# AnnaLew/pangenomix

Hardware: AMD Instinct MI355X
Metric: proteins/sec clustered at 0.8 identity + pan/core iters/sec, 400-genome set (higher is better)
Workload: dtype i32

## Files before the change

pangenomix_amd/csrc/cluster.hip:

```cpp
#include <algorithm>
#include <chrono>
#include <cstdlib>
#include <cmath>
#include <type_traits>
#include <functional>
#include <condition_variable>
#include <mutex>
#include <thread>
#include <vector>

#include "cluster_layout.h"
#include "cluster_resolve.h"
#include "cluster_tables.h"
#include "pgx_internal.h"

namespace {

using namespace pgxc;

constexpr uint32_t kWindowMax = 65536;
constexpr int kDiscoveryRounds = 2;
constexpr uint32_t kBlockCap = 4096;
constexpr uint32_t kBlockCapMin = 64;

constexpr uint32_t kMaxLen = 1u << 22;
constexpr uint32_t kPackedLenAa = 32767, kPackedLenNt = 16383;
constexpr uint32_t kSentinel = 0xFFFFFFFFu;
constexpr uint32_t kDiagLdsCap = 2048;
constexpr uint32_t kDiagLdsSmall = 512;
constexpr int kMaxBand = 64;

__constant__ int8_t kBlosum62_dev[kNAA1 * kNAA1] = PGXC_BLOSUM62_FLAT;

enum : uint32_t { E_TOUCHED = 1,
                  E_POOL = 2,
                  E_TABLE = 4,
                  E_BAND = 8,
                  E_PAIRS = 16,
                  E_WORDMULT = 32 };

struct PairSel {
    const uint32_t *d_begin, *d_end;
    uint32_t cap;
    const uint32_t *list;
    uint32_t n_list;
    const uint8_t *only_a, *only_not_b;
    uint8_t *accepted_out;
    uint32_t b0;
    uint32_t skip_evaluated;
    uint32_t all_if_le;
};
__device__ __forceinline__ uint32_t sel_count(const PairSel &s) {
    if (s.list) return s.n_list;
    uint32_t e = *s.d_end;
    if (e > s.cap) e = s.cap;
    const uint32_t b = s.d_begin ? *s.d_begin : 0u;
    return e > b ? e - b : 0u;
}
__device__ __forceinline__ uint32_t sel_pair(const PairSel &s, uint32_t w) {
    return s.list ? s.list[w] : (s.d_begin ? *s.d_begin : 0u) + w;
}

struct DevSeqs {
    const uint8_t *res;
    const uint64_t *off;
    const uint32_t *len;
    const uint32_t *wcode;
    const uint16_t *wmult;
    const uint32_t *wcnt;
    const uint32_t *pk;
    const uint32_t *pk_off;
    uint32_t n_fwd;
    int32_t base;
    int32_t kd;
    int32_t nt;
    uint32_t mshift;
};
__device__ __forceinline__ uint32_t entry_rmask(const DevSeqs &S) { return (1u << S.mshift) - 1u; }
__device__ __forceinline__ uint32_t entry_fmax(const DevSeqs &S) { return 0xFFFFFFFFu >> S.mshift; }
__device__ __forceinline__ uint32_t real_of(const DevSeqs &S, uint32_t k) { return k >= S.n_fwd ? k - S.n_fwd : k; }

__constant__ int8_t kAa2Idx_dev[26] = {0, 2, 4, 3, 6, 13, 7, 8, 9, 20, 11, 10, 12,
                                       2, 20, 14, 5, 1, 15, 16, 20, 19, 17, 20, 18, 6};

__device__ __forceinline__ bool is_letter(uint8_t ch) {
    ch &= 0xDF;
    return ch >= 'A' && ch <= 'Z';
}

__global__ __launch_bounds__(256) void seq_len_kernel(const uint8_t *__restrict__ res,
                                                     const uint64_t *__restrict__ off, uint32_t n, uint64_t total,
                                                     uint32_t *__restrict__ len) {
    const uint32_t lane = threadIdx.x & 63u;
    const uint32_t i = blockIdx.x * 4u + (threadIdx.x >> 6);
    if (i >= n) return;
    const uint64_t b = off[i], e = off[i + 1];
    uint32_t c = 0;
    const uint64_t a0 = b & ~3ull;
    for (uint64_t a = a0 + 4ull * lane; a < e; a += 256) {
        uint32_t word = 0;
        if (a + 4 <= total) word = *reinterpret_cast<const uint32_t *>(res + a);
        else for (uint64_t p = a; p < total; ++p) word |= (uint32_t)res[p] << (8 * (p - a));
#pragma unroll
        for (int t = 0; t < 4; ++t) {
            const uint64_t p = a + t;
            c += (p >= b && p < e) && is_letter((uint8_t)(word >> (8 * t)));
        }
    }
    for (int d = 32; d > 0; d >>= 1) c += __shfl_xor(c, d);
    if (lane == 0) len[i] = c;
}

__global__ __launch_bounds__(256) void encode_gather_kernel(const uint8_t *__restrict__ in,
                                                           const uint64_t *__restrict__ in_off,
                                                           const uint32_t *__restrict__ order,
                                                           const uint64_t *__restrict__ out_off,
                                                           uint8_t *__restrict__ out, uint32_t n, int nt) {
    const uint32_t lane = threadIdx.x & 63u;
    const uint32_t k = blockIdx.x * 4u + (threadIdx.x >> 6);
    if (k >= n) return;
    const uint32_t src = order[k];
    const uint64_t b = in_off[src], e = in_off[src + 1];
    uint64_t w = out_off[k];
    for (uint64_t q0 = b; q0 < e; q0 += 256) {
        uint8_t chs[4];
#pragma unroll
        for (int j = 0; j < 4; ++j) { const uint64_t p = q0 + 64u * j + lane; chs[j] = p < e ? in[p] : (uint8_t)0; }
#pragma unroll
        for (int j = 0; j < 4; ++j) {
            const uint8_t ch = chs[j];
            const bool ok = is_letter(ch);
            const unsigned long long m = __ballot(ok);
            if (ok) {
                const uint8_t up = ch & 0xDF;
                const uint8_t idx = nt ? (uint8_t)(up == 'A' ? 0 : up == 'C' ? 1 : up == 'G' ? 2 : (up == 'T' || up == 'U') ? 3 : 4)
                                       : (uint8_t)kAa2Idx_dev[up - 'A'];
                out[w + __popcll(m & ((1ull << lane) - 1ull))] = idx;
            }
            w += __popcll(m);
        }
    }
}

__global__ __launch_bounds__(256) void revcomp_kernel(uint8_t *__restrict__ res, const uint64_t *__restrict__ off,
                                                     const uint32_t *__restrict__ len, uint32_t n) {
    const uint32_t lane = threadIdx.x & 63u;
    const uint32_t k = blockIdx.x * 4u + (threadIdx.x >> 6);
    if (k >= n) return;
    const uint64_t src = off[k], dst = off[n + k];
    const uint32_t L = len[k];
    for (uint32_t i = lane; i < L; i += 64) {
        const uint8_t b = res[src + L - 1 - i];
        res[dst + i] = b < 4 ? (uint8_t)(3 - b) : b;
    }
}

__global__ __launch_bounds__(256) void pack5_kernel(const uint8_t *__restrict__ res, const uint64_t *__restrict__ off,
                                                   const uint32_t *__restrict__ len,
                                                   const uint32_t *__restrict__ pk_off, uint32_t n,
                                                   uint32_t *__restrict__ pk) {
    const uint32_t lane = threadIdx.x & 63u;
    const uint32_t k = blockIdx.x * 4u + (threadIdx.x >> 6);
    if (k >= n) return;
    const uint8_t *s = res + off[k];
    const uint32_t L = len[k], nw = (L + 5u) / 6u;
    uint32_t *dst = pk + pk_off[k];
    for (uint32_t w = lane; w < nw; w += 64) {
// ... 1070 lines not shown
    __shared__ uint32_t s_cnt[4][kMaxChunks];
    const uint32_t lane = threadIdx.x & 63u, n = *n_open;
    uint32_t *cnt = s_cnt[threadIdx.x >> 6];
    for (uint32_t w = blockIdx.x * 4 + (threadIdx.x >> 6); w < n; w += gridDim.x * 4) {
        const uint32_t k = ulist[w], ql = k - b0;
        if (decided[ql]) continue;
        const uint32_t c = chunk_of(C, ql);
        const int32_t t0 = req_aan[k];
        bool cand = false;
        for (uint32_t strand = 0; strand < (both ? 2u : 1u) && !cand; ++strand) {
            const uint32_t ks = strand ? S.n_fwd + k : k;
            const uint64_t o = S.off[ks];
            const uint32_t nw = S.wcnt[ks];
            if (lane < kMaxChunks) cnt[lane] = 0u;
            __builtin_amdgcn_fence(__ATOMIC_RELEASE, "workgroup");
            __builtin_amdgcn_wave_barrier();
            uint32_t sum = 0;
            for (uint32_t i = lane; i < nw; i += 64) {
                const uint32_t m = S.wmult[o + i];
                const uint32_t *rec = first + (size_t)S.wcode[o + i] * stride;
                for (uint32_t t4 = 0; t4 <= c; t4 += 4) {
                    uint32_t v[4];
                    if (stride >= 4) { const uint4 x = *reinterpret_cast<const uint4 *>(rec + t4); v[0] = x.x; v[1] = x.y; v[2] = x.z; v[3] = x.w; }
                    else { v[0] = rec[0]; v[1] = stride > 1 ? rec[1] : 0u; v[2] = 0u; v[3] = 0u; }
#pragma unroll
                    for (uint32_t j = 0; j < 4; ++j) {
                        const uint32_t t = t4 + j;
                        if (t > c || (v[j] >> 16) != epoch) continue;
                        if (t < c) atomicAdd(&cnt[t], m);
                        else if (65535u - (v[j] & 65535u) < ql) sum += m;
                    }
                }
            }
            for (int d = 32; d > 0; d >>= 1) sum += __shfl_xor(sum, d);
            __builtin_amdgcn_fence(__ATOMIC_RELEASE, "workgroup");
            __builtin_amdgcn_wave_barrier();
            __builtin_amdgcn_fence(__ATOMIC_ACQUIRE, "workgroup");
            uint32_t mx = lane < c ? cnt[lane] : 0u;
            mx = mx > sum ? mx : sum;
            for (int d = 32; d > 0; d >>= 1) { const uint32_t v = __shfl_xor(mx, d); mx = v > mx ? v : mx; }
            cand = mx != 0u && (int32_t)mx >= t0;
            __builtin_amdgcn_wave_barrier();
        }
        if (!cand && lane == 0) {
            done[ql] = 1;
            list[atomicAdd(n_list, 1u)] = k;
        }
    }
}

__global__ __launch_bounds__(256) void thresholds_kernel(const uint32_t *__restrict__ len, uint32_t n,
                                                        const int32_t *__restrict__ tab, uint32_t n_len,
                                                        int32_t *__restrict__ aa1, int32_t *__restrict__ aas,
                                                        int32_t *__restrict__ aan) {
    const uint32_t k = blockIdx.x * blockDim.x + threadIdx.x;
    if (k >= n) return;
    const uint32_t L = len[k];
    aa1[k] = tab[L]; aas[k] = tab[n_len + L]; aan[k] = tab[2 * n_len + L];
}


__global__ void retire_block_kernel(uint8_t *__restrict__ done, uint8_t *__restrict__ inblk, uint32_t nb, uint32_t final_,
                                    uint32_t *__restrict__ begin) {
    const uint32_t q = blockIdx.x * blockDim.x + threadIdx.x;
    if (q == 0 && begin) { begin[C_TOUCH] = 0u; begin[C_NK] = 0u; begin[C_EVAL0] = begin[C_NW]; }
    if (q < nb && inblk[q]) { done[q] = (uint8_t)final_; inblk[q] = 0; }
}
__global__ __launch_bounds__(256) void window_init_kernel(uint32_t *__restrict__ counters,
                                                         unsigned long long *__restrict__ best,
                                                         unsigned long long *__restrict__ rc_visits,
                                                         uint8_t *__restrict__ flags, uint32_t window_cap) {
    const uint32_t q = blockIdx.x * blockDim.x + threadIdx.x;
    if (q < C_COUNT && q != C_ERR) counters[q] = 0u;
    if (q >= window_cap) return;
    best[q] = kNoBest;
    if (rc_visits) rc_visits[q] = 0ull;
    if (q < 4 * window_cap / 8) reinterpret_cast<unsigned long long *>(flags)[q] = 0ull;
}

__global__ __launch_bounds__(256) void mark_absent_kernel(const uint8_t *__restrict__ taken, uint32_t nb,
                                                         uint8_t *__restrict__ done,
                                                         unsigned long long *__restrict__ best) {
    const uint32_t q = blockIdx.x * blockDim.x + threadIdx.x;
    if (q < nb && taken[q]) { done[q] = 2; best[q] = 0ull; }
}

__global__ __launch_bounds__(256) void min_rows_kernel(const unsigned long long *__restrict__ rows, uint32_t n_rows,
                                                      uint32_t row_stride, uint32_t n,
                                                      unsigned long long *__restrict__ out, uint32_t *__restrict__ err) {
    const uint32_t i = blockIdx.x * blockDim.x + threadIdx.x;
    if (i == 0) {
        uint32_t e = 0;
        for (uint32_t r = 0; r < n_rows; ++r) e |= (uint32_t)rows[(size_t)r * row_stride + PGX_EXCHANGE_KEYS];
        if (e) atomicOr(err, e);
    }
    if (i >= n) return;
    unsigned long long m = rows[i];
    for (uint32_t r = 1; r < n_rows; ++r) { const unsigned long long v = rows[(size_t)r * row_stride + i]; m = v < m ? v : m; }
    out[i] = m;
}

__global__ void exchange_prepare_kernel(const uint32_t *__restrict__ counters, uint32_t pair_cap,
                                        unsigned long long *__restrict__ send, uint32_t inject) {
    send[PGX_EXCHANGE_KEYS] = counters[C_ERR] | (counters[C_NW] > pair_cap ? (uint32_t)E_PAIRS : 0u) | inject;
}

constexpr uint32_t kPairWords = sizeof(Pair) / 4;
static_assert(sizeof(Pair) % 4 == 0, "pair records are published as dwords");
struct PubSeg { const uint32_t *src; uint32_t *dst; const uint32_t *count; uint32_t fixed, words, cap; };
constexpr int kPubSegs = 8;
struct PubArgs { PubSeg seg[kPubSegs]; int n; };
__global__ __launch_bounds__(256) void publish_kernel(PubArgs a) {
    for (int s = 0; s < a.n; ++s) {
        const PubSeg g = a.seg[s];
        uint32_t c = g.count ? *g.count : g.fixed;
        if (c > g.cap) c = g.cap;
        const uint32_t total = c * g.words;
        for (uint32_t i = blockIdx.x * blockDim.x + threadIdx.x; i < total; i += gridDim.x * blockDim.x) g.dst[i] = g.src[i];
    }
}

__global__ __launch_bounds__(256) void gather_pairs_kernel(const Pair *__restrict__ pairs,
                                                          const uint32_t *__restrict__ list, uint32_t n,
                                                          Pair *__restrict__ out) {
    const uint32_t i = blockIdx.x * blockDim.x + threadIdx.x;
    if (i < n) out[i] = pairs[list[i]];
}


__device__ __forceinline__ uint32_t wave_excl_scan(uint32_t v, uint32_t lane, uint32_t *total) {
    uint32_t x = v;
    for (int d = 1; d < 64; d <<= 1) {
        const uint32_t y = __shfl_up(x, d);
        if ((int)lane >= d) x += y;
    }
    *total = __shfl(x, 63);
    return x - v;
}

template <typename DiagPtr>
__device__ void band_from_histogram(DiagPtr d, int len1, int len2, int band_width, int required_aa1,
                                    double cluster_thd, int *best_sum, int *bl, int *bc, int *br) {
    const int lane = threadIdx.x & 63;
    const int nall = len1 + len2 - 1;
    const int band_b = required_aa1 - 1 >= 0 ? required_aa1 - 1 : 0;
    const int band_e = nall - band_b;
    const int band_m = band_b + band_width - 1 < band_e ? band_b + band_width - 1 : band_e;
    const int w = band_m - band_b + 1;
    const int T = band_e - band_m - 1 > 0 && w > 0 ? band_e - band_m - 1 : 0;
    using Cell = std::remove_cv_t<std::remove_reference_t<decltype(d[0])>>;
    constexpr int kHalf = (int)sizeof(Cell) * 4;
    auto hits = [&](int i) { return (int)(d[i] & ((Cell(1) << kHalf) - 1)); };
    auto weighted = [&](int i) { return (int)(d[i] >> kHalf); };
    auto wave_max = [&](int v) { for (int o = 32; o > 0; o >>= 1) v = max(v, __shfl_xor(v, o)); return v; };
    auto wave_min = [&](int v) { for (int o = 32; o > 0; o >>= 1) v = min(v, __shfl_xor(v, o)); return v; };
    auto wave_sum = [&](int v) { for (int o = 32; o > 0; o >>= 1) v += __shfl_xor(v, o); return v; };
    const int x0 = lane < w ? weighted(band_b + lane) : 0;
    const int score2_first = wave_sum(x0);
    int max_diag2 = wave_max(x0);
    int imax = max_diag2 > 0 ? wave_min(x0 == max_diag2 && lane < w ? band_b + lane : INT32_MAX) : 0;
    const int per = (T + 63) / 64;
    const int t_lo = 1 + lane * per, t_hi = min(T + 1, t_lo + per);
    auto window_at = [&](int t) {
        int sum = 0;
        for (int i = 0; i < w; ++i) sum += weighted(band_b + t + i);
        return sum;
    };
    int first = 0, local_max = INT32_MIN;
    if (t_lo < t_hi) {
        first = window_at(t_lo);
        int sc = first;
        local_max = sc;
        for (int t = t_lo + 1; t < t_hi; ++t) {
            sc += weighted(band_m + t) - weighted(band_b + t - 1);
            local_max = max(local_max, sc);
        }
    }
    int before = local_max;
    for (int o = 1; o < 64; o <<= 1) {
        const int up = __shfl_up(before, o);
        if (lane >= o) before = max(before, up);
    }
    before = __shfl_up(before, 1);
    before = max(lane == 0 ? INT32_MIN : before, score2_first);
    int last_t = 0, cand_val = 0, cand_t = INT32_MAX;
    if (t_lo < t_hi) {
        int sc = first, run = before;
        for (int t = t_lo; t < t_hi; ++t) {
            if (t > t_lo) sc += weighted(band_m + t) - weighted(band_b + t - 1);
            if (sc > run) {
                run = sc; last_t = t;
                const int v = weighted(band_m + t);
                if (v > cand_val) { cand_val = v; cand_t = t; }
            }
        }
    }
    const int best_t = wave_max(last_t);
    const int cand_best = wave_max(cand_val);
    if (cand_best > max_diag2) {
        max_diag2 = cand_best;
        imax = band_m + wave_min(cand_val == cand_best ? cand_t : INT32_MAX);
    }
    int from = band_b + best_t, end = band_m + best_t;
    int best_score = wave_sum(lane < w ? hits(from + lane) : 0);
    int mlen = imax;
    if (imax > len1) mlen = nall - imax;
    const int emax = (int)((1.0 - cluster_thd) * mlen) + 1;
    for (int j = from; j < imax; ++j) {
        const int s1 = hits(j);
        if ((imax - j) > emax || s1 < 1) { best_score -= s1; from++; } else break;
    }
    for (int j = end; j > imax; --j) {
        const int s1 = j >= band_b ? hits(j) : 0;
        if ((j - imax) > emax || s1 < 1) { best_score -= s1; end--; } else break;
    }
    *bl = from - len1 + 1; *br = end - len1 + 1; *bc = imax - len1 + 1; *best_sum = best_score;
}

__device__ __forceinline__ int kd_code(const DevSeqs &S, const uint8_t *__restrict__ s, int j, int *cpx) {
    int code = 0, c = 1;
    bool bad = false;
    for (int t = 0; t < S.kd; ++t) {
        const int r = s[j + t];
        bad |= r >= S.base;
        code = code * S.base + r;
        if (t) c += r != s[j + t - 1];
    }
    *cpx = c;
    return (S.nt && bad) ? -1 : code;
}

template <uint32_t CAP, typename Cell>
__global__ __launch_bounds__(64) void diag_kernel(DevSeqs S, const uint32_t *__restrict__ rep_seq,
                                                 Pair *__restrict__ pairs, PairSel sel,
                                                 const int32_t *__restrict__ req_aa1,
                                                 const int32_t *__restrict__ req_aas, int band_width,
                                                 double cluster_thd, uint32_t *__restrict__ gscratch,
                                                 uint32_t gscratch_stride, uint32_t gscratch_cells,
                                                 uint32_t *__restrict__ n_wide, uint32_t *__restrict__ err) {
    if (blockIdx.x == 0 && threadIdx.x == 0) *n_wide = 0u;
    constexpr bool kWideCell = sizeof(Cell) == 8;
    constexpr int kHalf = (int)sizeof(Cell) * 4;
    __shared__ Cell diag[CAP];
    __shared__ uint32_t taap[kNAA1 * kNAA1 + 7];
    __shared__ uint32_t abeg[kNAA1 * kNAA1 + 7];
    __shared__ uint16_t alist[CAP];
    constexpr uint32_t kRepCap = CAP * 3 / 2;
    __shared__ uint4 stage1[kWideCell ? 1 : CAP / 16 + 2];
    __shared__ uint4 stage2[kWideCell ? 1 : kRepCap / 16 + 2];
    const uint32_t lane = threadIdx.x;
    const uint32_t np = sel_count(sel);
    const int N2 = S.nt ? 256 : kNAA1 * kNAA1;
    for (uint32_t w = blockIdx.x; w < np; w += gridDim.x) {
        const uint32_t p = sel_pair(sel, w);
        const Pair pr = pairs[p];
        if (np > sel.all_if_le) {
            if (sel.only_a && !sel.only_a[pr.r - sel.b0]) continue;
            if (sel.only_not_b && sel.only_not_b[pr.r - sel.b0]) continue;
        }
        if (sel.skip_evaluated && (pr.flags & F_EVAL)) continue;
        const uint32_t k1 = pr.q, k2 = rep_seq ? rep_seq[pr.r] : pr.r;
        const uint32_t k1r = real_of(S, k1);
        const int len1 = (int)S.len[k1], len2 = (int)S.len[k2];
        const uint8_t *s1 = S.res + S.off[k1];
        const uint8_t *s2 = S.res + S.off[k2];
        const int nall = len1 + len2 - 1;
        const int d_lo = req_aa1[k1r] - 1 >= 0 ? req_aa1[k1r] - 1 : 0;
        const int d_hi = nall - d_lo;
        const int n_d = d_hi >= d_lo ? d_hi - d_lo + 1 : 0;
        const bool big = kWideCell || (uint32_t)n_d > CAP || (uint32_t)len1 > CAP;
        Cell *dg = big ? reinterpret_cast<Cell *>(gscratch + (size_t)blockIdx.x * gscratch_stride) : diag;
        uint32_t *al_big = big ? reinterpret_cast<uint32_t *>(dg + 2 * (size_t)gscratch_cells) : nullptr;
        const int last1 = len1 - S.kd, last2 = len2 - S.kd;
        const bool in_lds = !kWideCell && !big && (uint32_t)len2 <= kRepCap;
        if (in_lds) {
            const uint8_t *g1 = reinterpret_cast<const uint8_t *>(reinterpret_cast<uintptr_t>(s1) & ~uintptr_t(15));
            const uint8_t *g2 = reinterpret_cast<const uint8_t *>(reinterpret_cast<uintptr_t>(s2) & ~uintptr_t(15));
            const uint32_t sh1 = (uint32_t)(s1 - g1), sh2 = (uint32_t)(s2 - g2);
            const uint32_t nv1 = (sh1 + (uint32_t)len1 + 15u) / 16u, nv2 = (sh2 + (uint32_t)len2 + 15u) / 16u;
            uint4 v1[(CAP / 16 + 2 + 63) / 64], v2[(kRepCap / 16 + 2 + 63) / 64];
#pragma unroll
            for (uint32_t t = 0; t < sizeof(v1) / sizeof(uint4); ++t) if (lane + 64 * t < nv1) v1[t] = reinterpret_cast<const uint4 *>(g1)[lane + 64 * t];
#pragma unroll
            for (uint32_t t = 0; t < sizeof(v2) / sizeof(uint4); ++t) if (lane + 64 * t < nv2) v2[t] = reinterpret_cast<const uint4 *>(g2)[lane + 64 * t];
            constexpr uint32_t kEnd = 0xFFFFu;
            uint32_t *head = taap;
            uint16_t *next = alist;
            for (int i = lane; i < n_d; i += 64) diag[i] = Cell(0);
            for (int c = lane; c < N2; c += 64) head[c] = kEnd;
#pragma unroll
            for (uint32_t t = 0; t < sizeof(v1) / sizeof(uint4); ++t) if (lane + 64 * t < nv1) stage1[lane + 64 * t] = v1[t];
#pragma unroll
            for (uint32_t t = 0; t < sizeof(v2) / sizeof(uint4); ++t) if (lane + 64 * t < nv2) stage2[lane + 64 * t] = v2[t];
            __syncthreads();
            const uint8_t *l1 = reinterpret_cast<const uint8_t *>(stage1) + sh1;
            const uint8_t *l2 = reinterpret_cast<const uint8_t *>(stage2) + sh2;
            for (int j = lane; j <= last1; j += 64) {
                int cpx;
                const int c = kd_code(S, l1, j, &cpx);
                if (c >= 0) next[j] = (uint16_t)atomicExch(&head[c], (uint32_t)j);
            }
            __syncthreads();
            for (int i = lane; i <= last2; i += 64) {
                int cpx;
                const int c = kd_code(S, l2, i, &cpx);
                if (c < 0) continue;
                const Cell inc = Cell(1) | (Cell((uint32_t)cpx) << kHalf);
                for (uint32_t j = head[c]; j != kEnd; j = next[j]) {
                    const int d = len1 - 1 + i - (int)j;
                    if (d >= d_lo && d <= d_hi) atomicAdd(&diag[d - d_lo], inc);
                }
            }
            __syncthreads();
        } else {
        for (int i = lane; i < n_d; i += 64) dg[i] = Cell(0);
        for (int c = lane; c < N2; c += 64) taap[c] = 0u;
        __syncthreads();
        for (int j = lane; j <= last1; j += 64) {
            int cpx;
            const int c = kd_code(S, s1, j, &cpx);
            if (c >= 0) atomicAdd(&taap[c], 1u);
        }
        __syncthreads();
        {
            uint32_t loc[7], sum = 0;
            for (int t = 0; t < 7; ++t) { const int c = lane * 7 + t; loc[t] = c < N2 ? taap[c] : 0u; sum += loc[t]; }
            uint32_t total, base = wave_excl_scan(sum, lane, &total);
            for (int t = 0; t < 7; ++t) { const int c = lane * 7 + t; if (c < N2) { abeg[c] = base; taap[c] = 0u; } base += loc[t]; }
        }
        __syncthreads();
        for (int j = lane; j <= last1; j += 64) {
            int cpx;
            const int c = kd_code(S, s1, j, &cpx);
            if (c < 0) continue;
            const uint32_t pos = abeg[c] + atomicAdd(&taap[c], 1u);
            if (big) al_big[pos] = (uint32_t)j; else alist[pos] = (uint16_t)j;
        }
        __syncthreads();
        for (int i = lane; i <= last2; i += 64) {
            int cpx;
            const int c = kd_code(S, s2, i, &cpx);
            if (c < 0) continue;
            const Cell inc = Cell(1) | (Cell((uint32_t)cpx) << kHalf);
            const uint32_t b = abeg[c], e = b + taap[c];
            for (uint32_t t = b; t < e; ++t) {
                const int j = big ? (int)al_big[t] : (int)alist[t];
                const int d = len1 - 1 + i - j;
                if (d >= d_lo && d <= d_hi) atomicAdd(&dg[d - d_lo], inc);
            }
        }
        __syncthreads();
        }
        int best_sum, bl, bc, br;
        {
            const int bw = band_width < len1 + len2 - 2 ? band_width : len1 + len2 - 2;
            if (in_lds) band_from_histogram(diag - d_lo, len1, len2, bw, req_aa1[k1r], cluster_thd, &best_sum, &bl, &bc, &br);
            else band_from_histogram(dg - d_lo, len1, len2, bw, req_aa1[k1r], cluster_thd, &best_sum, &bl, &bc, &br);
        }
        if (lane == 0) {
            uint32_t fl = F_EVAL;
            if (best_sum >= req_aas[k1r]) fl |= F_DIAG_PASS;
            if (!(br >= len2 || bl <= -len1 || bl > br)) fl |= F_BAND_OK;
            if (br - bl + 1 > kMaxBand) { fl |= F_TOO_BIG; if (fl & F_DIAG_PASS) atomicOr(err, (uint32_t)E_BAND); }
            pairs[p].best_sum = best_sum; pairs[p].band_left = bl; pairs[p].band_center = bc;
            pairs[p].band_right = br; pairs[p].flags = fl;
        }
        __syncthreads();
    }
}

enum { BK_NONE = 0, BK_DIAG = 1, BK_LEFT = 2, BK_TOP = 3 };

__device__ __forceinline__ int64_t shfl_i64(int64_t v, int src_lane) {
    const int lo = __shfl((int)(uint32_t)v, src_lane);
    const int hi = __shfl((int)(v >> 32), src_lane);
    return (int64_t)(((uint64_t)(uint32_t)hi << 32) | (uint32_t)lo);
}

__device__ int band_align_wave(const uint8_t *__restrict__ s1, const uint8_t *__restrict__ s2, int len1,
                               int len2, int bl, int bc, int br, const int8_t *__restrict__ sub ,
                               int gap_open, int gap_ext) {
    const int lane = threadIdx.x & 63;
    const int bw = br - bl + 1;
    const int j1 = lane;
    const bool col = j1 < bw;
    const int i_start = max(1, 1 - bl - j1);
    const int i_end = min(len1, len2 - bl - j1);
    const int i_start_left = max(1, 2 - bl - j1);
    const int maxd = bc - bl;
    const int dist = j1 > maxd ? j1 - maxd : maxd - j1;
    const int64_t bonus = 4 - (dist & 3);
    const int64_t gap = kScoreScale * gap_open, ext = kScoreScale * gap_ext;
    int64_t sc = 0;
    int bk = BK_NONE, id = 0;
    const int t_last = 2 * len1 + bw - 1;
    for (int t = 2; t <= t_last; ++t) {
        const int64_t l_sc_n = shfl_i64(sc, (lane + 63) & 63);
        const int l_meta = __shfl((id << 2) | bk, (lane + 63) & 63);
        const int64_t r_sc_n = shfl_i64(sc, (lane + 1) & 63);
        const int r_meta = __shfl((id << 2) | bk, (lane + 1) & 63);
        const int d = t - j1;
        const int i = d >> 1;
        if (col && !(d & 1) && i >= i_start && i <= i_end) {
            const int j = j1 + i + bl;
            const int ci = s1[i - 1], cj = s2[j - 1];
            int64_t sij = kScoreScale * (int64_t)sub[ci * kNAA1 + cj];
            if (sij > 0) sij += bonus;
            int64_t p_sc; int p_id;
            if (i - 1 >= i_start) { p_sc = sc; p_id = id; }
            else { p_sc = ext * (int64_t)((i - 1 == 0) ? (j - 1) : (i - 1)); p_id = 0; }
            int64_t best = p_sc + sij;
            int back = BK_DIAG, nid = p_id + (ci == cj);
            const int64_t gap0 = (i == len1 || j == len2) ? ext : gap;
            if (j1 > 0) {
                int64_t l_sc; int l_bk, l_id;
                if (i >= i_start_left) { l_sc = l_sc_n; l_bk = l_meta & 3; l_id = l_meta >> 2; }
                else { l_sc = ext * (int64_t)i; l_bk = BK_NONE; l_id = 0; }
                const int64_t s = l_sc + (l_bk == BK_LEFT ? ext : gap0);
                if (s > best) { best = s; back = BK_LEFT; nid = l_id; }
            }
            if (j1 + 1 < bw) {
                int64_t r_sc; int r_bk, r_id;
                if (i - 1 >= 1) { r_sc = r_sc_n; r_bk = r_meta & 3; r_id = r_meta >> 2; }
                else { r_sc = ext * (int64_t)j; r_bk = BK_NONE; r_id = 0; }
                const int64_t s = r_sc + (r_bk == BK_TOP ? ext : gap0);
                if (s > best) { best = s; back = BK_TOP; nid = r_id; }
            }
            sc = best; bk = back; id = nid;
        }
    }
    int end_lane;
    if (len2 - bl < len1) end_lane = 0;
    else if (len1 + br < len2) end_lane = bw - 1;
    else end_lane = len2 - len1 - bl;
    return __shfl(id, end_lane);
}

constexpr int kA16MaxSlot = 4096;
constexpr int kA16BigSlot = 8192;
constexpr int kScaleShift = 14;

__device__ __forceinline__ int dpp_row_shr1(int v) { return __builtin_amdgcn_update_dpp(0, v, 0x111, 0xF, 0xF, true); }
__device__ __forceinline__ int dpp_row_shl1(int v) { return __builtin_amdgcn_update_dpp(0, v, 0x101, 0xF, 0xF, true); }

__device__ __forceinline__ uint32_t lane_select(uint64_t mask, uint32_t if_set, uint32_t if_clear) {
    uint32_t d;
    asm("v_cndmask_b32_e64 %0, %1, %2, %3" : "=v"(d) : "v"(if_clear), "v"(if_set), "s"(mask));
    return d;
}
__device__ __forceinline__ uint64_t lanes_equal(uint32_t a, uint32_t b) { return __builtin_amdgcn_uicmp(a, b, 32 ); }

__device__ __forceinline__ bool pair_is_wide(int len1, int len2, int bl, int br, int max_sum) {
    return len1 + len2 > max_sum || br - bl + 1 > 32;
}

template <int kA16Slot>
__global__ __launch_bounds__(256) void align16_kernel(DevSeqs S, const uint32_t *__restrict__ rep_seq,
                                                     Pair *__restrict__ pairs, PairSel sel,
                                                     const int32_t *__restrict__ req_aa1, double cluster_thd,
                                                     uint32_t b0, unsigned long long *__restrict__ best,
                                                     uint32_t key_flag, uint32_t *__restrict__ n_wide, uint32_t second_pass) {
    __shared__ int2 tab[4][kNAA1 * kNAA1];
    __shared__ uint32_t seqbuf[16 * (kA16Slot / 4) + 32];
    __builtin_amdgcn_s_setprio(3);
    const uint32_t n = sel_count(sel);
    if (blockIdx.x * 16u >= n) return;
    if (second_pass && *n_wide == 0u) return;
    for (int c = threadIdx.x; c < 4 * kNAA1 * kNAA1; c += 256) {
        const int cc = c % (kNAA1 * kNAA1);
        const int s = S.nt ? (cc / kNAA1 == cc % kNAA1 ? 2 : -2) : (int)kBlosum62_dev[cc];
        const int v = s * (1 << kScaleShift) + (s > 0 ? c / (kNAA1 * kNAA1) + 1 : 0);
        tab[c / (kNAA1 * kNAA1)][cc] = make_int2(v * 4 + 2, cc / kNAA1 == cc % kNAA1);
    }
    __syncthreads();
    const int lane = threadIdx.x & 63, gl = lane & 15;
    const int slot = (threadIdx.x >> 6) * 4 + (lane >> 4);
    const uint8_t *sb = reinterpret_cast<const uint8_t *>(seqbuf + slot * (kA16Slot / 4));
    const int gap = (S.nt ? -6 : kGapOpen) * (1 << kScaleShift), ext = (S.nt ? -1 : kGapExt) * (1 << kScaleShift);
    constexpr int kNever = INT32_MIN / 2;

    for (uint32_t base = blockIdx.x * 16u; base < n; base += gridDim.x * 16u) {
        const uint32_t w = base + (uint32_t)slot;
        uint32_t p = 0;
        Pair pr{};
        bool fast = false;
        int len1 = 1, len2 = 1;
        uint32_t k1 = 0, k2 = 0;
        if (w < n) {
            p = sel_pair(sel, w);
            pr = pairs[p];
            k1 = pr.q; k2 = rep_seq ? rep_seq[pr.r] : pr.r;
            len1 = (int)S.len[k1]; len2 = (int)S.len[k2];
            fast = (pr.flags & (F_DIAG_PASS | F_BAND_OK | F_TOO_BIG | F_ALIGNED)) == (F_DIAG_PASS | F_BAND_OK);
            if (fast && pair_is_wide(len1, len2, pr.band_left, pr.band_right, kA16Slot - 96)) {
// ... 428 lines not shown
    int pool_cur = 0;
    uint64_t pool_cap = 0;
    uint32_t epoch_idx = 0;
    uint32_t epoch_tag = 0;
    double cur_frac = 0.0;
    uint64_t chunk_words = 0;
    uint64_t pending_words = 0;
    PendingWindow pending;
    DevBuf d_res, d_off, d_len, d_wcode, d_wmult, d_wcnt, d_aa1, d_aas, d_aan, d_lines, d_pool[2], d_idx, d_newbits, d_touched,
        d_first, d_rcvis, d_visits, d_pairsK, d_blk_list, d_ulist, d_new_list, d_order, d_list, d_gather, d_pk, d_pkoff, d_thr,
        d_hugewords, d_xsend, d_xrecv,
        d_hist, d_sortcnt, d_tilesum, d_runs, d_in_len;
    WindowSet sets[2];
    unsigned long long *x_send = nullptr;
    const unsigned long long *x_recv = nullptr;
    HostVec<uint32_t> h_hist, order, h_len, h_wcnt;
    HostVec<uint64_t> h_off, h_runs;
    HostVec<int32_t> h_thr;
    HostVec<int32_t> cluster_of;
    HostVec<int32_t> iden_of;
    HostVec<uint8_t> strand_of;
    Pinned<Pair> hK, h_gather;
    Pinned<unsigned long long> h_rcvis;
    Pinned<uint32_t> h_cnt, h_blk, h_new, h_list, h_push;
    Pinned<uint8_t> h_taken;
    std::vector<uint32_t> rep_seq;
    std::vector<uint32_t> members;
    std::vector<uint8_t> status;
    std::vector<unsigned long long> winner_key;
    std::vector<uint32_t> order_k, rank_of, bucket_k, fill_k, flight;
    pgx_cluster_stats S{};
    uint64_t gpu_pairs = 0, gpu_aligned = 0, gpu_aligned_bytes = 0, filter_walk_words = 0;
    uint64_t visits_rc = 0, n_rounds = 0, n_blocks = 0;
    int inject_rank = -1;
    uint64_t inject_at = 0, n_exchanges = 0;

    ClusterCall(pgx_ctx *c, const pgx_cluster_params *p, hipStream_t stream)
        : ctx(c), P(p), st_main(stream),
          d_res(c, CL_SLOT_RES), d_off(c, CL_SLOT_OFF), d_len(c, CL_SLOT_LEN), d_wcode(c, CL_SLOT_WCODE), d_wmult(c, CL_SLOT_WMULT),
          d_wcnt(c, CL_SLOT_WCNT), d_aa1(c, CL_SLOT_AA1), d_aas(c, CL_SLOT_AAS), d_aan(c, CL_SLOT_AAN), d_lines(c, CL_SLOT_LINES),
          d_pool{{c, CL_SLOT_POOL0}, {c, CL_SLOT_POOL1}}, d_idx(c, CL_SLOT_IDX), d_newbits(c, CL_SLOT_NEWBITS),
          d_touched(c, CL_SLOT_TOUCHED), d_first(c, CL_SLOT_FIRST), d_rcvis(c, CL_SLOT_RCVIS), d_visits(c, CL_SLOT_VISITS),
          d_pairsK(c, CL_SLOT_PAIRS_K), d_blk_list(c, CL_SLOT_BLK_LIST), d_ulist(c, CL_SLOT_ULIST), d_new_list(c, CL_SLOT_NEW_LIST),
          d_order(c, CL_SLOT_ORDER), d_list(c, CL_SLOT_LIST), d_gather(c, CL_SLOT_GATHER), d_pk(c, CL_SLOT_PK),
          d_pkoff(c, CL_SLOT_PKOFF), d_thr(c, CL_SLOT_THR), d_hugewords(c, CL_SLOT_HUGEWORDS), d_xsend(c, CL_SLOT_XSEND),
          d_xrecv(c, CL_SLOT_XRECV), d_hist(c, CL_SLOT_HIST), d_sortcnt(c, CL_SLOT_SORTCNT), d_tilesum(c, CL_SLOT_TILESUM),
          d_runs(c, CL_SLOT_RUNS), d_in_len(c, CL_SLOT_IN_LEN),
          sets{{c, CL_SLOT_COUNTERS, CL_SLOT_BEST_OWN, CL_SLOT_FLAGS, CL_SLOT_PAIRS_W, CL_SLOT_GSCRATCH, CL_PIN_W, CL_PIN_BEST, CL_PIN_CCNT},
               {c, CL_SLOT_COUNTERS2, CL_SLOT_BEST2, CL_SLOT_FLAGS2, CL_SLOT_PAIRS_W2, CL_SLOT_GSCRATCH2, CL_PIN_W2, CL_PIN_BEST2, CL_PIN_CCNT2}},
          hK(c, CL_PIN_K), h_gather(c, CL_PIN_GATHER), h_rcvis(c, CL_PIN_RCVIS), h_cnt(c, CL_PIN_CNT), h_blk(c, CL_PIN_BLK),
          h_new(c, CL_PIN_NEW), h_list(c, CL_PIN_LIST), h_push(c, CL_PIN_PUSH), h_taken(c, CL_PIN_TAKEN) {
        nt = P->alphabet == 1;
        both = nt && P->both_strands != 0;
        native_exchange = !P->exchange && P->shard_count >= 1 && ctx->comm;
        exchanging = P->exchange || native_exchange;
        shard_count = P->shard_count > 0 ? (uint32_t)P->shard_count : 1u;
        shard_index = P->shard_count > 0 ? (uint32_t)P->shard_index : 0u;
        count_replicated = shard_index == 0;
        overlap = !nt && !std::getenv("PGX_NO_OVERLAP");
        const char *tr = std::getenv("PGX_TRACE");
        trace = tr != nullptr;
        trace2 = trace && tr[0] == '2';
        sets[0].st = st_main;
        sets[1].st = ctx->stream2;
        t_call0 = t_loop0 = Clock::now();
    }
    void phase(const char *what) {
        if (!trace) return;
        const double now = 1e3 * seconds_since(t_call0);
        fprintf(stderr, "[pgx] %-28s %8.2f ms\n", what, now - t_mark);
        t_mark = now;
    }
    void give_stats(pgx_cluster_stats *stats) const { if (stats) *stats = S; }
};

struct Window {
    uint32_t b0 = 0, nb = 0, ns = 0;
    bool sweep = false;
    bool mark_absent = false;
    int set = 0;
    uint32_t n_reps = 0;
    uint64_t window_words = 0, blocks_before = 0;
    int two_len = 0, a16_slot = 0;
    uint32_t *d_poolp = nullptr;
    Chunks chunks;
    FilterArgs FA{};
    Clock::time_point t_sweep0;
    bool older_reps = false;
    uint32_t n_listed = 0;
    uint32_t n_struck = 0;
    bool strike_recorded = false;
    uint32_t nW = 0;
};

double chunk_frac_default() {
    static const double chunk_frac = std::getenv("PGX_CHUNK_FRAC") ? std::atof(std::getenv("PGX_CHUNK_FRAC")) : 0.8;
    return chunk_frac;
}


int ensure_pool(ClusterCall &C, uint64_t entries, hipStream_t on) {
    const uint64_t need = 8 * entries + 4096;
    if (need <= C.pool_cap) return PGX_OK;
    if (need > 0xFFFFFFF0ull) { pgx_set_error("pgx_cluster_greedy: word index too large for 32-bit pool offsets"); return PGX_ERR_CAPACITY; }
    const uint64_t want = std::min<uint64_t>(0xFFFFFFF0ull, need + need / 2);
    DevBuf &nb_ = C.d_pool[C.pool_cur ^ 1];
    PGX_HIP(nb_.alloc(want * 4));
    if (C.pool_cap) PGX_HIP(hipMemcpyAsync(nb_.p, C.d_pool[C.pool_cur].p, C.pool_cap * 4, hipMemcpyDeviceToDevice, on));
    C.pool_cur ^= 1;
    C.pool_cap = want;
    return PGX_OK;
}

uint32_t form_window(const ClusterCall &C, uint32_t b0, Chunks &chunks, uint32_t limit) {
    return pgxc::form_window(C.h_len.data(), b0, limit, C.window_cap, C.chunking, C.chunk_words, chunks);
}

void account(ClusterCall &C, const Pair *pp, uint32_t cnt) {
    for (uint32_t i = 0; i < cnt; ++i) {
        ++C.gpu_pairs;
        if (!pair_is_aligned(pp[i])) continue;
        ++C.gpu_aligned;
        C.gpu_aligned_bytes += C.h_len[pp[i].q] + C.h_len[pp[i].r];
    }
}

void add_counts(pgx_cluster_stats &S, const PairCounts &c) {
    S.filter_pairs += c.filter_pairs; S.aligned_pairs += c.aligned_pairs;
    S.aligned_rep_len += c.aligned_rep_len; S.dp_cells += c.dp_cells;
}

void window_error(const ClusterCall &C, uint32_t e, uint32_t at) {
    pgx_set_error("pgx_cluster_greedy: capacity failure in the window at %u%s:%s%s%s%s%s%s", at,
                  C.exchanging ? " (on this or another process)" : "",
                  e & E_TOUCHED ? " append scratch list full;" : "", e & E_POOL ? " overflow pool of the word index full;" : "",
                  e & E_TABLE ? " exact table of the filter overflowed;" : "",
                  e & E_BAND ? " alignment band wider than 64 diagonals;" : "", e & E_PAIRS ? " candidate pair buffer overflow;" : "",
                  e & E_WORDMULT ? " a word occurs more than 65535 times in one sequence;" : "");
}

int band_error() {
    pgx_set_error("pgx_cluster_greedy: alignment band wider than %d diagonals", kMaxBand);
    return PGX_ERR_CAPACITY;
}

int evaluate(ClusterCall &C, WindowSet &ws, Window &W, Pair *pairs, const PairSel &sel, unsigned long long *best_arr,
             uint32_t grid_hint) {
    const pgx_cluster_params *P = C.P;
    const uint32_t dg = grid_hint ? std::min(C.diag_grid, grid_hint) : C.diag_grid;
    const uint32_t ag = grid_hint ? std::min(kAlignGrid, (grid_hint + 15) / 16) : kAlignGrid;
    const uint32_t len0 = C.h_len[W.b0];
    {
        ProfScope prof(C.ctx, "diag_kernel", ws.st);
        auto kern = len0 > C.packed_len ? diag_kernel<64, unsigned long long>
                    : (len0 <= kDiagLdsSmall ? diag_kernel<kDiagLdsSmall, uint32_t>
                       : (len0 <= 2 * kDiagLdsSmall ? diag_kernel<2 * kDiagLdsSmall, uint32_t> : diag_kernel<kDiagLdsCap, uint32_t>));
        kern<<<dg, 64, 0, ws.st>>>(C.DS, nullptr, pairs, sel, C.d_aa1.as<int32_t>(), C.d_aas.as<int32_t>(),
                                   P->band_width, P->identity, ws.d_gs, C.gs_stride, C.gs_cells, ws.dc + C_WIDE, ws.dc + C_ERR);
    }
    LAUNCH_CHECK();
    {
        ProfScope prof(C.ctx, "align_kernel", ws.st);
        const int a16_slot = W.a16_slot, two_len = W.two_len;
        auto kern = a16_slot == 1024 ? align16_kernel<1024> : (a16_slot == 1536 ? align16_kernel<1536> : (a16_slot == 2048 ? align16_kernel<2048>
                    : (a16_slot == 3072 ? align16_kernel<3072> : align16_kernel<kA16MaxSlot>)));
        kern<<<ag, 256, 0, ws.st>>>(C.DS, nullptr, pairs, sel, C.d_aa1.as<int32_t>(), P->identity, W.b0, best_arr, 0u, ws.dc + C_WIDE, 0u);
        const bool big_pass = a16_slot == kA16MaxSlot && two_len > kA16MaxSlot - 96;
        const bool may_be_wide = W.older_reps || two_len > a16_slot - 96 || P->band_width > 32;
        if (big_pass)
            align16_kernel<kA16BigSlot><<<ag, 256, 0, ws.st>>>(C.DS, nullptr, pairs, sel, C.d_aa1.as<int32_t>(), P->identity, W.b0, best_arr,
                                                               0u, ws.dc + C_WIDE, 1u);
        if (may_be_wide)
            align_kernel<<<grid_hint ? std::min(kAlignGrid, (grid_hint + 3) / 4) : kAlignGrid, 256, 0, ws.st>>>(
                C.DS, nullptr, pairs, sel, C.d_aa1.as<int32_t>(), P->identity, W.b0, best_arr, 0u, 1, (big_pass ? kA16BigSlot : a16_slot) - 96, ws.dc + C_WIDE);
    }
    LAUNCH_CHECK();
    return PGX_OK;
}

int exchange_best(ClusterCall &C, WindowSet &ws, Window &W) {
    if (!C.exchanging) return PGX_OK;
    const pgx_cluster_params *P = C.P;
    ++C.n_exchanges;
    exchange_prepare_kernel<<<1, 1, 0, ws.st>>>(ws.dc, C.pair_cap, ws.d_best,
                                                C.inject_rank == (int)C.shard_index && C.inject_at == C.n_exchanges ? (uint32_t)E_PAIRS : 0u);
    if (C.native_exchange) {
        const int rc = pgx_rccl_all_gather_u64(C.ctx, C.x_send + (size_t)W.set * PGX_EXCHANGE_WORDS,
                                               const_cast<unsigned long long *>(C.x_recv) + (size_t)W.set * C.shard_count * PGX_EXCHANGE_WORDS,
                                               PGX_EXCHANGE_WORDS, ws.st);
        if (rc) return rc;
    } else if (P->exchange(P->exchange_user, (void *)ws.st, W.set) != 0) {
        pgx_set_error("pgx_cluster_greedy: the exchange callback failed in the window at %u", W.b0);
        return PGX_ERR_INTERNAL;
    }
    min_rows_kernel<<<(W.nb + 255) / 256, 256, 0, ws.st>>>(
        C.x_recv + (size_t)W.set * C.shard_count * PGX_EXCHANGE_WORDS,
        C.shard_count, PGX_EXCHANGE_WORDS, W.nb, ws.d_best, ws.dc + C_ERR);
    LAUNCH_CHECK();
    return PGX_OK;
}

int evaluate_round(ClusterCall &C, WindowSet &ws, Window &W) {
    const PairSel sel{ws.dc + C_EVAL0, ws.dc + C_NW, C.pair_cap, nullptr, 0, nullptr, nullptr, nullptr, W.b0, 0, 0};
    int rc = evaluate(C, ws, W, ws.pairsW, sel, ws.d_best, 0);
    if (rc) return rc;
    return exchange_best(C, ws, W);
}

int index_append(ClusterCall &C, WindowSet &ws, Window &W, const uint32_t *list, const uint32_t *d_lo, const uint32_t *d_hi) {
    ++C.epoch_idx;
    uint32_t *const map = C.d_newbits.as<uint32_t>() + (size_t)(C.epoch_idx & 1u) * C.bm_words;
    uint32_t *const next_map = C.d_newbits.as<uint32_t>() + (size_t)((C.epoch_idx + 1u) & 1u) * C.bm_words;
    ProfScope prof(C.ctx, "index_append", ws.st);
    index_append_kernel<<<512, 256, 0, ws.st>>>(C.DS, list, d_lo, d_hi, C.d_lines.as<IndexLine>(), C.epoch_idx,
                                                map, W.b0, W.nb, C.d_touched.as<Deferred>(),
                                                ws.dc + C_TOUCH, (uint32_t)C.max_window_words, ws.dc + C_ERR);
    index_grow_kernel<<<256, 256, 0, ws.st>>>(C.d_lines.as<IndexLine>(), W.d_poolp, C.d_idx.as<uint32_t>(),
                                              (uint32_t)C.pool_cap, C.d_touched.as<Deferred>(), ws.dc + C_TOUCH,
                                              (uint32_t)C.max_window_words, ws.dc + C_ERR);
    index_place_kernel<<<256, 256, 0, ws.st>>>(C.d_lines.as<IndexLine>(), W.d_poolp, C.d_touched.as<Deferred>(),
                                               ws.dc + C_TOUCH, (uint32_t)C.max_window_words, reinterpret_cast<uint4 *>(next_map),
                                               C.bm_words / 4);
    LAUNCH_CHECK();
    return PGX_OK;
}

int filter_new_and_evaluate(ClusterCall &C, WindowSet &ws, Window &W, const uint32_t *d_lo, const uint32_t *d_hi) {
    FilterArgs F = W.FA;
    F.epoch = C.epoch_idx; F.d_round_lo = d_lo; F.d_round_hi = d_hi;
    F.newbits = C.d_newbits.as<uint32_t>() + (size_t)(C.epoch_idx & 1u) * C.bm_words;
    {
        ProfScope prof(C.ctx, "filter_kernel<new>", ws.st);
        auto kern = C.nt ? filter_kernel<true, true> : filter_kernel<false, true>;
        kern<<<std::min(kFilterGrid, (W.ns + 3) / 4), 256, 0, ws.st>>>(C.DS, F);
    }
    LAUNCH_CHECK();
    C.filter_walk_words += W.window_words * (C.both ? 2 : 1) / C.shard_count;
    return evaluate_round(C, ws, W);
}

int wait_closed(ClusterCall &C, PendingWindow &pw) {
    WindowSet &ws = C.sets[pw.set];
    if (C.overlap) {
        const auto t0 = Clock::now();
        hipError_t e;
        while ((e = hipEventQuery(ws.post)) == hipErrorNotReady) {
        }
        g_wait_s += seconds_since(t0);
        PGX_HIP(e);
    } else {
        PGX_HIP(spin_sync(ws.st));
    }
    pw.nW = pw.h_ccnt->p[C_NW];
    if (pw.h_ccnt->p[C_ERR]) { window_error(C, pw.h_ccnt->p[C_ERR], pw.b0); return PGX_ERR_CAPACITY; }
    if (pw.nW > C.pair_cap) {
        pgx_set_error("pgx_cluster_greedy: candidate pair buffer overflow (%u > %u) in the window at %u", pw.nW, C.pair_cap, pw.b0);
        return PGX_ERR_CAPACITY;
    }
    if (pw.nW > pw.hW->cap) {
        PGX_HIP(pw.hW->reserve(pw.nW));
        PGX_HIP(hipMemcpyAsync(pw.hW->p, ws.pairsW, (size_t)pw.nW * sizeof(Pair), hipMemcpyDeviceToHost, ws.st));
        PGX_HIP(spin_sync(ws.st));
    }
    return PGX_OK;
}

int finish_window(ClusterCall &C, PendingWindow &pw) {
    if (C.overlap) { int rc = wait_closed(C, pw); if (rc) return rc; }
    const uint32_t b0 = pw.b0, nb = pw.nb, n = C.n;
    pgx_cluster_stats &S = C.S;
    uint8_t *const status = C.status.data();
    unsigned long long *const winner_key = C.winner_key.data();
    C.pending_words = 0;
    for (uint32_t q = 0; q < nb; ++q) {
        if (status[q] != ST_OPEN) continue;
        const unsigned long long key = pw.h_best->p[q];
        if (key == kNoBest) {
            if (pw.sweep) { status[q] = ST_NONE; continue; }
            pgx_set_error("pgx_cluster_greedy: unresolved member after the last block"); return PGX_ERR_INTERNAL;
        }
        status[q] = ST_MEMBER;
        winner_key[q] = key;
        C.strand_of[b0 + q] = (uint8_t)(key >> 63);
        if (pw.sweep) C.h_taken.p[b0 + q] = 1;
    }
    if (C.both)
        for (uint32_t q = 0; q < nb; ++q)
            if (status[q] == ST_REP || status[q] == ST_NONE || (status[q] == ST_MEMBER && (winner_key[q] >> 63))) C.visits_rc += C.h_rcvis.p[q];
    for (uint32_t q = 0; q < nb; ++q)
        if (status[q] == ST_REP) {
            C.cluster_of[b0 + q] = (int32_t)C.rep_seq.size();
            C.rep_seq.push_back(b0 + q);
            S.sum_len_reps += C.h_len[b0 + q];
            S.rep_words += C.h_wcnt[b0 + q];
        }
    for (uint32_t q = 0; q < nb; ++q)
        if (status[q] == ST_MEMBER) C.cluster_of[b0 + q] = C.cluster_of[(uint32_t)winner_key[q] & 0x7FFFFFFFu];
    account(C, pw.hW->p, pw.nW);
    PairCounts examined;
    const bool fits = finish_window_pairs(pw.hW->p, pw.nW, b0, n, status, winner_key, C.h_len.data(), C.iden_of.data(), examined);
    add_counts(S, examined);
    if (!fits) return band_error();
    C.members.resize(C.rep_seq.size(), 0u);
    for (uint32_t q = 0; q < nb; ++q) {
        if (status[q] == ST_ABSENT || status[q] == ST_NONE) continue;
        const uint32_t k = b0 + q, o = C.order[k];
        const int32_t c = C.cluster_of[k];
        C.out_cluster[o] = c;
        C.out_member[o] = (int32_t)C.members[(size_t)c]++;
// ... 824 lines not shown
```

Baseline: 16.60 million.

## Use DPP wave reductions, parallel band trimming, and NT-specialized kd_code in diag kernel

Replaces the shuffle-based wave sum/max/min and prefix-max scans in band_from_histogram with DPP-based primitives from a new wave_dpp.h header. Turns the serial per-diagonal band-trimming loops into wave-parallel loops that use ballot to find the first diagonal that stays. Also specializes diag_kernel and kd_code on nucleotide vs protein input at compile time, removing the runtime k-mer length loop. The aim is to cut reduction latency and serial scalar work per pair, at the cost of more template instantiations and hardware-specific DPP control codes.

```diff
diff --git a/pangenomix_amd/csrc/cluster.hip b/pangenomix_amd/csrc/cluster.hip
--- a/pangenomix_amd/csrc/cluster.hip
+++ b/pangenomix_amd/csrc/cluster.hip
@@ -13,6 +13,7 @@
 #include "cluster_resolve.h"
 #include "cluster_tables.h"
 #include "pgx_internal.h"
+#include "wave_dpp.h"
 
 namespace {
 
@@ -1389,13 +1390,10 @@
     constexpr int kHalf = (int)sizeof(Cell) * 4;
     auto hits = [&](int i) { return (int)(d[i] & ((Cell(1) << kHalf) - 1)); };
     auto weighted = [&](int i) { return (int)(d[i] >> kHalf); };
-    auto wave_max = [&](int v) { for (int o = 32; o > 0; o >>= 1) v = max(v, __shfl_xor(v, o)); return v; };
-    auto wave_min = [&](int v) { for (int o = 32; o > 0; o >>= 1) v = min(v, __shfl_xor(v, o)); return v; };
-    auto wave_sum = [&](int v) { for (int o = 32; o > 0; o >>= 1) v += __shfl_xor(v, o); return v; };
     const int x0 = lane < w ? weighted(band_b + lane) : 0;
-    const int score2_first = wave_sum(x0);
-    int max_diag2 = wave_max(x0);
-    int imax = max_diag2 > 0 ? wave_min(x0 == max_diag2 && lane < w ? band_b + lane : INT32_MAX) : 0;
+    const int score2_first = wave_dpp::sum(x0);
+    int max_diag2 = wave_dpp::max(x0);
+    int imax = max_diag2 > 0 ? wave_dpp::min(x0 == max_diag2 && lane < w ? band_b + lane : INT32_MAX) : 0;
     const int per = (T + 63) / 64;
     const int t_lo = 1 + lane * per, t_hi = min(T + 1, t_lo + per);
     auto window_at = [&](int t) {
@@ -1413,13 +1411,7 @@
             local_max = max(local_max, sc);
         }
     }
-    int before = local_max;
-    for (int o = 1; o < 64; o <<= 1) {
-        const int up = __shfl_up(before, o);
-        if (lane >= o) before = max(before, up);
-    }
-    before = __shfl_up(before, 1);
-    before = max(lane == 0 ? INT32_MIN : before, score2_first);
+    const int before = max(wave_dpp::shift_up1(INT32_MIN, wave_dpp::prefix_max(local_max)), score2_first);
     int last_t = 0, cand_val = 0, cand_t = INT32_MAX;
     if (t_lo < t_hi) {
         int sc = first, run = before;
@@ -1432,42 +1424,56 @@
             }
         }
     }
-    const int best_t = wave_max(last_t);
-    const int cand_best = wave_max(cand_val);
+    const int best_t = wave_dpp::max(last_t);
+    const int cand_best = wave_dpp::max(cand_val);
     if (cand_best > max_diag2) {
         max_diag2 = cand_best;
-        imax = band_m + wave_min(cand_val == cand_best ? cand_t : INT32_MAX);
+        imax = band_m + wave_dpp::min(cand_val == cand_best ? cand_t : INT32_MAX);
     }
     int from = band_b + best_t, end = band_m + best_t;
-    int best_score = wave_sum(lane < w ? hits(from + lane) : 0);
+    int best_score = wave_dpp::sum(lane < w ? hits(from + lane) : 0);
     int mlen = imax;
     if (imax > len1) mlen = nall - imax;
     const int emax = (int)((1.0 - cluster_thd) * mlen) + 1;
-    for (int j = from; j < imax; ++j) {
-        const int s1 = hits(j);
-        if ((imax - j) > emax || s1 < 1) { best_score -= s1; from++; } else break;
-    }
-    for (int j = end; j > imax; --j) {
-        const int s1 = j >= band_b ? hits(j) : 0;
-        if ((j - imax) > emax || s1 < 1) { best_score -= s1; end--; } else break;
+    for (;;) {
+        const int j = from + lane;
+        const bool in = j < imax;
+        const int s1 = in ? hits(j) : 0;
+        const unsigned long long stay = __ballot(!(in && ((imax - j) > emax || s1 < 1)));
+        const int n = stay ? __ffsll(stay) - 1 : 64;
+        const int drop = lane < n ? s1 : 0;
+        if (__ballot(drop != 0)) best_score -= wave_dpp::sum(drop);
+        from += n;
+        if (n < 64) break;
+    }
+    for (;;) {
+        const int j = end - lane;
+        const bool in = j > imax;
+        const int s1 = in && j >= band_b ? hits(j) : 0;
+        const unsigned long long stay = __ballot(!(in && ((j - imax) > emax || s1 < 1)));
+        const int n = stay ? __ffsll(stay) - 1 : 64;
+        const int drop = lane < n ? s1 : 0;
+        if (__ballot(drop != 0)) best_score -= wave_dpp::sum(drop);
+        end -= n;
+        if (n < 64) break;
     }
     *bl = from - len1 + 1; *br = end - len1 + 1; *bc = imax - len1 + 1; *best_sum = best_score;
 }
 
-__device__ __forceinline__ int kd_code(const DevSeqs &S, const uint8_t *__restrict__ s, int j, int *cpx) {
-    int code = 0, c = 1;
-    bool bad = false;
-    for (int t = 0; t < S.kd; ++t) {
-        const int r = s[j + t];
-        bad |= r >= S.base;
-        code = code * S.base + r;
-        if (t) c += r != s[j + t - 1];
-    }
-    *cpx = c;
-    return (S.nt && bad) ? -1 : code;
-}
-
-template <uint32_t CAP, typename Cell>
+template <bool NT>
+__device__ __forceinline__ int kd_code(const uint8_t *__restrict__ s, int j, int *cpx) {
+    if constexpr (NT) {
+        const int r0 = s[j], r1 = s[j + 1], r2 = s[j + 2], r3 = s[j + 3];
+        *cpx = 1 + (r1 != r0) + (r2 != r1) + (r3 != r2);
+        return ((r0 | r1 | r2 | r3) >= 4) ? -1 : ((r0 * 4 + r1) * 4 + r2) * 4 + r3;
+    } else {
+        const int r0 = s[j], r1 = s[j + 1];
+        *cpx = 1 + (r1 != r0);
+        return r0 * kNAA1 + r1;
+    }
+}
+
+template <uint32_t CAP, typename Cell, bool NT>
 __global__ __launch_bounds__(64) void diag_kernel(DevSeqs S, const uint32_t *__restrict__ rep_seq,
                                                  Pair *__restrict__ pairs, PairSel sel,
                                                  const int32_t *__restrict__ req_aa1,
@@ -1487,7 +1493,7 @@
     __shared__ uint4 stage2[kWideCell ? 1 : kRepCap / 16 + 2];
     const uint32_t lane = threadIdx.x;
     const uint32_t np = sel_count(sel);
-    const int N2 = S.nt ? 256 : kNAA1 * kNAA1;
+    constexpr int N2 = NT ? 256 : kNAA1 * kNAA1, KD = NT ? 4 : 2;
     for (uint32_t w = blockIdx.x; w < np; w += gridDim.x) {
         const uint32_t p = sel_pair(sel, w);
         const Pair pr = pairs[p];
@@ -1508,7 +1514,7 @@
         const bool big = kWideCell || (uint32_t)n_d > CAP || (uint32_t)len1 > CAP;
         Cell *dg = big ? reinterpret_cast<Cell *>(gscratch + (size_t)blockIdx.x * gscratch_stride) : diag;
         uint32_t *al_big = big ? reinterpret_cast<uint32_t *>(dg + 2 * (size_t)gscratch_cells) : nullptr;
-        const int last1 = len1 - S.kd, last2 = len2 - S.kd;
+        const int last1 = len1 - KD, last2 = len2 - KD;
         const bool in_lds = !kWideCell && !big && (uint32_t)len2 <= kRepCap;
         if (in_lds) {
             const uint8_t *g1 = reinterpret_cast<const uint8_t *>(reinterpret_cast<uintptr_t>(s1) & ~uintptr_t(15));
@@ -1534,13 +1540,13 @@
             const uint8_t *l2 = reinterpret_cast<const uint8_t *>(stage2) + sh2;
             for (int j = lane; j <= last1; j += 64) {
                 int cpx;
-                const int c = kd_code(S, l1, j, &cpx);
+                const int c = kd_code<NT>(l1, j, &cpx);
                 if (c >= 0) next[j] = (uint16_t)atomicExch(&head[c], (uint32_t)j);
             }
             __syncthreads();
             for (int i = lane; i <= last2; i += 64) {
                 int cpx;
-                const int c = kd_code(S, l2, i, &cpx);
+                const int c = kd_code<NT>(l2, i, &cpx);
                 if (c < 0) continue;
                 const Cell inc = Cell(1) | (Cell((uint32_t)cpx) << kHalf);
                 for (uint32_t j = head[c]; j != kEnd; j = next[j]) {
@@ -1555,7 +1561,7 @@
         __syncthreads();
         for (int j = lane; j <= last1; j += 64) {
             int cpx;
-            const int c = kd_code(S, s1, j, &cpx);
+            const int c = kd_code<NT>(s1, j, &cpx);
             if (c >= 0) atomicAdd(&taap[c], 1u);
         }
         __syncthreads();
@@ -1568,7 +1574,7 @@
         __syncthreads();
         for (int j = lane; j <= last1; j += 64) {
             int cpx;
-            const int c = kd_code(S, s1, j, &cpx);
+            const int c = kd_code<NT>(s1, j, &cpx);
             if (c < 0) continue;
             const uint32_t pos = abeg[c] + atomicAdd(&taap[c], 1u);
             if (big) al_big[pos] = (uint32_t)j; else alist[pos] = (uint16_t)j;
@@ -1576,7 +1582,7 @@
         __syncthreads();
         for (int i = lane; i <= last2; i += 64) {
             int cpx;
-            const int c = kd_code(S, s2, i, &cpx);
+            const int c = kd_code<NT>(s2, i, &cpx);
             if (c < 0) continue;
             const Cell inc = Cell(1) | (Cell((uint32_t)cpx) << kHalf);
             const uint32_t b = abeg[c], e = b + taap[c];
@@ -2311,9 +2317,13 @@
     const uint32_t len0 = C.h_len[W.b0];
     {
         ProfScope prof(C.ctx, "diag_kernel", ws.st);
-        auto kern = len0 > C.packed_len ? diag_kernel<64, unsigned long long>
-                    : (len0 <= kDiagLdsSmall ? diag_kernel<kDiagLdsSmall, uint32_t>
-                       : (len0 <= 2 * kDiagLdsSmall ? diag_kernel<2 * kDiagLdsSmall, uint32_t> : diag_kernel<kDiagLdsCap, uint32_t>));
+        auto pick = [&](auto nt) {
+            constexpr bool NT = decltype(nt)::value;
+            return len0 > C.packed_len ? diag_kernel<64, unsigned long long, NT>
+                   : (len0 <= kDiagLdsSmall ? diag_kernel<kDiagLdsSmall, uint32_t, NT>
+                      : (len0 <= 2 * kDiagLdsSmall ? diag_kernel<2 * kDiagLdsSmall, uint32_t, NT> : diag_kernel<kDiagLdsCap, uint32_t, NT>));
+        };
+        auto kern = C.DS.nt ? pick(std::true_type{}) : pick(std::false_type{});
         kern<<<dg, 64, 0, ws.st>>>(C.DS, nullptr, pairs, sel, C.d_aa1.as<int32_t>(), C.d_aas.as<int32_t>(),
                                    P->band_width, P->identity, ws.d_gs, C.gs_stride, C.gs_cells, ws.dc + C_WIDE, ws.dc + C_ERR);
     }
diff --git a/pangenomix_amd/csrc/wave_dpp.h b/pangenomix_amd/csrc/wave_dpp.h
--- /dev/null
+++ b/pangenomix_amd/csrc/wave_dpp.h
@@ -0,0 +1,43 @@
+#pragma once
+#include <hip/hip_runtime.h>
+#include <stdint.h>
+
+namespace wave_dpp {
+
+template <int CTRL> __device__ __forceinline__ int dpp_all(int v) { return __builtin_amdgcn_update_dpp(0, v, CTRL, 0xF, 0xF, true); }
+template <int CTRL, int ROW_MASK = 0xF> __device__ __forceinline__ int dpp_or(int ident, int v) {
+    return __builtin_amdgcn_update_dpp(ident, v, CTRL, ROW_MASK, 0xF, false);
+}
+
+template <typename Op> __device__ __forceinline__ int reduce(int v, Op op) {
+    v = op(v, dpp_all<0xB1>(v));
+    v = op(v, dpp_all<0x4E>(v));
+    v = op(v, dpp_all<0x124>(v));
+    v = op(v, dpp_all<0x128>(v));
+    const int r0 = __builtin_amdgcn_readlane(v, 0), r1 = __builtin_amdgcn_readlane(v, 16);
+    const int r2 = __builtin_amdgcn_readlane(v, 32), r3 = __builtin_amdgcn_readlane(v, 48);
+    return op(op(r0, r1), op(r2, r3));
+}
+
+__device__ __forceinline__ int sum(int v) { return reduce(v, [](int a, int b) { return a + b; }); }
+__device__ __forceinline__ int max(int v) { return reduce(v, [](int a, int b) { return a > b ? a : b; }); }
+__device__ __forceinline__ int min(int v) { return reduce(v, [](int a, int b) { return a < b ? a : b; }); }
+__device__ __forceinline__ uint32_t sum(uint32_t v) { return (uint32_t)sum((int)v); }
+__device__ __forceinline__ uint32_t max(uint32_t v) {
+    return (uint32_t)reduce((int)v, [](int a, int b) { return (uint32_t)a > (uint32_t)b ? a : b; });
+}
+
+__device__ __forceinline__ int prefix_max(int v) {
+    auto mx = [](int a, int b) { return a > b ? a : b; };
+    v = mx(v, dpp_or<0x111>(INT32_MIN, v));
+    v = mx(v, dpp_or<0x112>(INT32_MIN, v));
+    v = mx(v, dpp_or<0x114>(INT32_MIN, v));
+    v = mx(v, dpp_or<0x118>(INT32_MIN, v));
+    v = mx(v, dpp_or<0x142, 0xA>(INT32_MIN, v));
+    v = mx(v, dpp_or<0x143, 0xC>(INT32_MIN, v));
+    return v;
+}
+
+__device__ __forceinline__ int shift_up1(int first, int v) { return dpp_or<0x138>(first, v); }
+
+}
```

After: 16.85 million (median of 6 runs). 1.5% higher.
